# wenhao728/VORTA

Hardware: NVIDIA B200
Metric: dit_denoise_step_ms (lower is better)
Workload: dtype bf16

## Files before the change

include/vorta_b200.h:

```cpp
#ifndef VORTA_B200_H_
#define VORTA_B200_H_

#include <stdint.h>

#ifdef __cplusplus
extern "C" {
#endif

#define VB_OK 0
#define VB_ERR_INVALID (-1)
#define VB_ERR_CUDA (-2)
#define VB_ERR_UNSUPPORTED (-3)

#define VB_BRANCH_FULL 0
#define VB_BRANCH_CORESET 1
#define VB_BRANCH_SLIDING 2
#define VB_BRANCH_SKIP (-1)
#define VB_BRANCH_FULL_LO 3
#define VB_BRANCH_FULL_HI 4
#define VB_BRANCH_FULL_PART(k, n) (16 + 8 * (n) + (k))

#define VB_DTYPE_F32 0
#define VB_DTYPE_BF16 1

// ... 90 lines not shown
int64_t vb_attn_workspace_bytes(const vb_plan* plan, int32_t batch, int32_t heads);
int vb_attn_fwd(vb_plan* plan, const vb_attn_args* args, vb_stream_t stream);

int vb_attn_dense(const void* q, const void* k, const void* v, void* out, const int64_t* q_stride,
                  const int64_t* k_stride, const int64_t* v_stride, const int64_t* out_stride, int32_t batch,
                  int32_t heads, int32_t n_q, int32_t n_k, vb_stream_t stream);

void vb_stats_reset(void);
int64_t vb_stats_launches(void);
double vb_stats_attn_flops(void);

int vb_block_ln_modulate(const void* x, const float* weight, const float* bias, const float* scale, const float* shift,
                         void* out, int64_t rows, int32_t dim, int32_t rows_per_batch, float eps, vb_stream_t stream);
int vb_block_gate_residual(const void* x, const void* y, const float* gate, void* out, int64_t rows, int32_t dim,
                           int32_t rows_per_batch, vb_stream_t stream);
int vb_block_rmsnorm_rope(const void* x, const void* weight, const float* cos_tab, const float* sin_tab, void* out,
                          int64_t rows, int32_t dim, int32_t tokens_per_batch, float eps, vb_stream_t stream);

int vb_block_headnorm_rope(const void* x, const void* weight, const float* cos_tab, const float* sin_tab, void* out,
                           int32_t batch, int32_t rows, int32_t heads, int32_t rope_rows, int32_t dst_rows,
                           int32_t dst_row0, float eps, vb_stream_t stream);

void vb_timing_enable(int on);
int vb_timing_collect(double* kernel_ms, int64_t* launches, double* flops);
#define VB_TIMING_ROUTED 0
#define VB_TIMING_DENSE 1
#define VB_TIMING_KINDS 2
int vb_timing_collect_kinds(double* kernel_ms, int64_t* launches, double* flops);

int vb_ulysses_pack_heads(const void* x, void* send, int32_t s_loc, int32_t heads, int32_t world, int32_t n_tensors,
// ... 18 lines not shown
```

vorta_b200/_lib.py:

```python
from __future__ import annotations

import ctypes as C
import os
import subprocess
from typing import Optional

_HERE = os.path.dirname(os.path.abspath(__file__))
LIB_PATH = os.environ.get("VB_LIB_PATH") or os.path.join(_HERE, "lib", "libvorta_b200.so")
CSRC_DIR = os.path.join(_HERE, "csrc")

VB_OK = 0
VB_ERR_INVALID = -1
VB_ERR_CUDA = -2
VB_ERR_UNSUPPORTED = -3

BRANCH_FULL, BRANCH_CORESET, BRANCH_SLIDING, BRANCH_SKIP = 0, 1, 2, -1
BRANCH_FULL_LO, BRANCH_FULL_HI = 3, 4
DTYPE_F32, DTYPE_BF16 = 0, 1
ATTN_CORESET_KV_FROM_K = 1


def branch_full_part(k: int, n: int) -> int:
    return 16 + 8 * n + k


(PLAN_SEQ_LEN, PLAN_NUM_GROUPS, PLAN_GROUP_SIZE, PLAN_CORESET_LEN, PLAN_NUM_TILES, PLAN_TILE_TOKENS,
 PLAN_NUM_POOLED, PLAN_KEYS_PER_QUERY, PLAN_SLIDING_PAIRS, PLAN_SLIDING_RUNS) = range(10)
(EXPORT_CENTER_INDICES, EXPORT_MARGIN_INDICES, EXPORT_TILE_MAP, EXPORT_TILE_WINDOW, EXPORT_SLIDING_RUNS,
 EXPORT_SLIDING_ITEMS, EXPORT_SLIDING_QUERY_MAP) = range(7)

EXPORTED_SYMBOLS = (
    "vb_last_error", "vb_version", "vb_device_check",
    "vb_plan_create", "vb_plan_destroy", "vb_plan_set_text_valid", "vb_plan_query", "vb_plan_export",
    "vb_router_forward", "vb_coreset_select", "vb_coreset_tables", "vb_gather_rows",
    "vb_attn_workspace_bytes", "vb_attn_fwd", "vb_attn_dense",
    "vb_block_ln_modulate", "vb_block_gate_residual", "vb_block_rmsnorm_rope", "vb_block_headnorm_rope",
    "vb_stats_reset", "vb_stats_launches", "vb_stats_attn_flops", "vb_timing_enable", "vb_timing_collect",
    "vb_timing_collect_kinds",
    "vb_ulysses_pack_heads", "vb_ulysses_pack_qkv", "vb_ulysses_unpack_heads", "vb_ulysses_scatter_qkv_slots",
)


class PlanDesc(C.Structure):
    _fields_ = [
        ("latent", C.c_int32 * 3),
        ("tile", C.c_int32 * 3),
        ("window", C.c_int32 * 3),
        ("lowres_window", C.c_int32 * 3),
        ("n_unpooled", C.c_int32),
        ("text_len", C.c_int32),
        ("text_valid", C.c_int32),
# ... 63 lines not shown
    lib.vb_attn_dense.argtypes = [vp, vp, vp, vp, C.POINTER(i64), C.POINTER(i64), C.POINTER(i64), C.POINTER(i64),
                                  i32, i32, i32, i32, vp]
    lib.vb_gather_rows.restype = C.c_int
    lib.vb_gather_rows.argtypes = [vp, i64, i64, i64, vp, i64, i64, i64, vp, i64, i64, i32, i32, i32, vp]
    lib.vb_attn_workspace_bytes.restype = i64
    lib.vb_attn_workspace_bytes.argtypes = [vp, i32, i32]
    lib.vb_attn_fwd.restype = C.c_int
    lib.vb_attn_fwd.argtypes = [vp, C.POINTER(AttnArgs), vp]
    lib.vb_stats_reset.restype = None
    lib.vb_stats_launches.restype = i64
    lib.vb_stats_attn_flops.restype = C.c_double
    lib.vb_block_ln_modulate.restype = C.c_int
    lib.vb_block_ln_modulate.argtypes = [vp, vp, vp, vp, vp, vp, i64, i32, i32, f32, vp]
    lib.vb_block_gate_residual.restype = C.c_int
    lib.vb_block_gate_residual.argtypes = [vp, vp, vp, vp, i64, i32, i32, vp]
    lib.vb_block_rmsnorm_rope.restype = C.c_int
    lib.vb_block_rmsnorm_rope.argtypes = [vp, vp, vp, vp, vp, i64, i32, i32, f32, vp]
    lib.vb_block_headnorm_rope.restype = C.c_int
    lib.vb_block_headnorm_rope.argtypes = [vp, vp, vp, vp, vp, i32, i32, i32, i32, i32, i32, f32, vp]
    lib.vb_timing_enable.restype = None
    lib.vb_timing_enable.argtypes = [C.c_int]
    lib.vb_timing_collect.restype = C.c_int
    lib.vb_timing_collect.argtypes = [C.POINTER(C.c_double), C.POINTER(i64), C.POINTER(C.c_double)]
    lib.vb_timing_collect_kinds.restype = C.c_int
    lib.vb_timing_collect_kinds.argtypes = [C.POINTER(C.c_double), C.POINTER(i64), C.POINTER(C.c_double)]
    lib.vb_ulysses_pack_heads.restype = C.c_int
    lib.vb_ulysses_pack_heads.argtypes = [vp, vp, i32, i32, i32, i32, i64, i64, C.POINTER(i32), vp]
    lib.vb_ulysses_pack_qkv.restype = C.c_int
    lib.vb_ulysses_pack_qkv.argtypes = [vp, vp, vp, C.POINTER(i64), C.POINTER(i64), vp, i32, i32, i32, C.POINTER(i32), vp]
    lib.vb_ulysses_scatter_qkv_slots.restype = C.c_int
# ... 27 lines not shown
```

vorta_b200/csrc/vb_api.cu:

```cuda
#include <math.h>
#include <stdlib.h>
#include <string.h>

#include <algorithm>
#include <array>
#include <map>
#include <vector>

#include <nvtx3/nvToolsExt.h>

#include "vb_common.cuh"

namespace vb {

struct NvtxRange {
  explicit NvtxRange(const char* name) { nvtxRangePushA(name); }
  ~NvtxRange() { nvtxRangePop(); }
};

static thread_local char g_err[512] = "";
void set_error(const char* fmt, ...) {
  va_list ap;
  va_start(ap, fmt);
  vsnprintf(g_err, sizeof(g_err), fmt, ap);
// ... 13 lines not shown

int launch_coreset_select(const SelectParams& p, cudaStream_t stream);
int launch_gather_rows(const GatherParams& p, cudaStream_t stream);
int launch_coreset_tables(const TablesParams& p, cudaStream_t stream);
int launch_zero_rows(__nv_bfloat16* out, int64_t sb, int64_t sh, int64_t ss, int batch, int heads, int row0,
                     int n_rows, cudaStream_t stream);
int launch_router(const void* temb, int temb_dtype, const void* w, const void* bias, int w_dtype,
                  int64_t w_layer_stride, int64_t bias_layer_stride, int n_layers, int batch, int embed_dim,
                  int heads, float tau, float* scores, int32_t* branch, cudaStream_t stream);
int launch_ulysses_permute(const void* src, void* dst, int s_loc, int heads, int world, int n_tensors,
                           int64_t src_tensor_stride, int64_t dst_tensor_stride, int pack, const int32_t* head_at,
                           cudaStream_t stream);
int launch_ulysses_pack_qkv(const void* q, const void* k, const void* v, const int64_t* stride_s,
                            const int64_t* stride_h, void* send, int s_loc, int heads, int world,
                            const int32_t* head_at, cudaStream_t stream);
int launch_ln_modulate(const void* x, const float* w, const float* b, const float* scale, const float* shift, void* out,
                       int64_t rows, int dim, int rows_per_batch, float eps, cudaStream_t stream);
int launch_gate_residual(const void* x, const void* y, const float* gate, void* out, int64_t rows, int dim,
                         int rows_per_batch, cudaStream_t stream);
int launch_rmsnorm_rope(const void* x, const void* weight, const float* cs, const float* sn, void* out, int64_t rows,
                        int dim, int tokens_per_batch, float eps, cudaStream_t stream);
int launch_headnorm_rope(const void* x, const void* weight, const float* cs, const float* sn, void* out, int batch,
                         int rows, int heads, int rope_rows, int dst_rows, int dst_row0, float eps,
                         cudaStream_t stream);
int launch_ulysses_scatter_slots(const void* q, const void* k, const void* v, const int64_t* stride_s,
                                 const int64_t* stride_h, void* const* peer_qkv, int64_t rows_total, int s_loc, int slots,
                                 int world, int rank, const int32_t* entry_peer, const int32_t* entry_slot,
                                 const int32_t* entry_head, int n_entries, cudaStream_t stream);
int make_qkv_tensor_map(CUtensorMap* map, const void* base, int64_t n_rows, int64_t heads, int64_t batch,
                        int64_t stride_b, int64_t stride_h, int64_t stride_s);
int launch_attn(const AttnTmaps& tmaps, const AttnParams& params, int n_ctas, cudaStream_t stream);

// ... 169 lines not shown
  pl->full.finalize();
  pl->coreset.finalize();
  pl->sliding.finalize();
  if (pl->has_device) {
    int rc;
    if ((rc = pl->full.upload()) != VB_OK) return rc;
    if ((rc = pl->coreset.upload()) != VB_OK) return rc;
    if ((rc = pl->sliding.upload()) != VB_OK) return rc;
  }
  return VB_OK;
}

extern "C" {

const char* vb_last_error(void) { return get_error(); }
int vb_version(void) { return 101; }

int vb_device_check(void) {
  int dev = 0, major = 0, minor = 0, count = 0;
  if (cudaGetDeviceCount(&count) != cudaSuccess || count == 0) {
    cudaGetLastError();
    set_error("no CUDA device: vorta_b200 has no CPU path");
    return VB_ERR_UNSUPPORTED;
  }
  VB_CUDA_OK(cudaGetDevice(&dev));
  VB_CUDA_OK(cudaDeviceGetAttribute(&major, cudaDevAttrComputeCapabilityMajor, dev));
  VB_CUDA_OK(cudaDeviceGetAttribute(&minor, cudaDevAttrComputeCapabilityMinor, dev));
  VB_REQUIRE(major == 10, VB_ERR_UNSUPPORTED, "device is sm_%d%d; this library is built for sm_100a only", major,
             minor);
  return VB_OK;
}
// ... 712 lines not shown
  }
  Output o;
  memset(&o, 0, sizeof(o));
  o.ptr = static_cast<__nv_bfloat16*>(out);
  for (int i = 0; i < 3; ++i) o.stride[i] = out_stride[i];
  Segment sg = segment_of(q, k, v, q_stride, k_stride, v_stride, n_q, n_k, heads, *sched);
  for (int h = 0; h < heads; ++h) sg.heads.push_back(AttnHead{h, h, 0});
  NvtxRange nvtx("vb_attn_dense");
  return launch_segments(&sg, 1, batch, o, nullptr, nullptr, VB_TIMING_DENSE, static_cast<cudaStream_t>(stream_));
}

int vb_block_ln_modulate(const void* x, const float* weight, const float* bias, const float* scale, const float* shift,
                         void* out, int64_t rows, int32_t dim, int32_t rows_per_batch, float eps, vb_stream_t stream) {
  VB_REQUIRE(x && out, VB_ERR_INVALID, "null argument");
  VB_REQUIRE((scale == nullptr) == (shift == nullptr), VB_ERR_INVALID, "scale and shift come together");
  int rc = launch_ln_modulate(x, weight, bias, scale, shift, out, rows, dim, rows_per_batch, eps,
                              static_cast<cudaStream_t>(stream));
  if (rc == VB_OK) ++g_launches;
  return rc;
}
int vb_block_gate_residual(const void* x, const void* y, const float* gate, void* out, int64_t rows, int32_t dim,
                           int32_t rows_per_batch, vb_stream_t stream) {
  VB_REQUIRE(x && y && out, VB_ERR_INVALID, "null argument");
  int rc = launch_gate_residual(x, y, gate, out, rows, dim, rows_per_batch, static_cast<cudaStream_t>(stream));
  if (rc == VB_OK) ++g_launches;
  return rc;
}
int vb_block_rmsnorm_rope(const void* x, const void* weight, const float* cos_tab, const float* sin_tab, void* out,
                          int64_t rows, int32_t dim, int32_t tokens_per_batch, float eps, vb_stream_t stream) {
  VB_REQUIRE(x && weight && out, VB_ERR_INVALID, "null argument");
  VB_REQUIRE((cos_tab == nullptr) == (sin_tab == nullptr), VB_ERR_INVALID, "cos and sin tables come together");
// ... 103 lines not shown
```

vorta_b200/csrc/vb_block.cu:

```cuda
#include "vb_common.cuh"

namespace vb {

constexpr int kRowThreads = 256;
constexpr int kMaxVec = 4;

__device__ __forceinline__ void unpack8(const uint4& v, float (&f)[8]) {
  const uint32_t w[4] = {v.x, v.y, v.z, v.w};
#pragma unroll
  for (int i = 0; i < 4; ++i) {
    f[2 * i + 0] = __uint_as_float(w[i] << 16);
    f[2 * i + 1] = __uint_as_float(w[i] & 0xffff0000u);
  }
}
__device__ __forceinline__ uint32_t pack2(float lo, float hi) {
  uint32_t r;
  asm("cvt.rn.bf16x2.f32 %0, %1, %2;" : "=r"(r) : "f"(hi), "f"(lo));
  return r;
}
__device__ __forceinline__ uint4 pack8(const float (&f)[8]) {
  return make_uint4(pack2(f[0], f[1]), pack2(f[2], f[3]), pack2(f[4], f[5]), pack2(f[6], f[7]));
}
__device__ __forceinline__ void block_sum2(float& a, float& b) {
  __shared__ float red[2][kRowThreads / 32];
#pragma unroll
  for (int o = 16; o >= 1; o >>= 1) {
    a += __shfl_xor_sync(0xffffffffu, a, o);
    b += __shfl_xor_sync(0xffffffffu, b, o);
  }
  const int w = threadIdx.x >> 5, l = threadIdx.x & 31;
  if (l == 0) { red[0][w] = a; red[1][w] = b; }
  __syncthreads();
  a = l < kRowThreads / 32 ? red[0][l] : 0.f;
  b = l < kRowThreads / 32 ? red[1][l] : 0.f;
#pragma unroll
  for (int o = 4; o >= 1; o >>= 1) {
    a += __shfl_xor_sync(0xffffffffu, a, o);
    b += __shfl_xor_sync(0xffffffffu, b, o);
  }
  a = __shfl_sync(0xffffffffu, a, 0);
  b = __shfl_sync(0xffffffffu, b, 0);
  __syncthreads();
}

__global__ void __launch_bounds__(kRowThreads)
vb_ln_modulate_kernel(const __nv_bfloat16* __restrict__ x, const float* __restrict__ w, const float* __restrict__ b,
                      const float* __restrict__ scale, const float* __restrict__ shift, __nv_bfloat16* __restrict__ out,
                      int dim, int rows_per_batch, float eps) {
  const int64_t row = blockIdx.x;
  const int nvec = dim >> 3;
  const uint4* xr = reinterpret_cast<const uint4*>(x + row * dim);
  float v[kMaxVec][8];
  float s1 = 0.f, s2 = 0.f;
#pragma unroll
  for (int i = 0; i < kMaxVec; ++i) {
    const int idx = threadIdx.x + i * kRowThreads;
    if (idx < nvec) {
      unpack8(xr[idx], v[i]);
#pragma unroll
      for (int e = 0; e < 8; ++e) { s1 += v[i][e]; s2 += v[i][e] * v[i][e]; }
    }
  }
  block_sum2(s1, s2);
  const float mean = s1 / dim;
  const float rstd = rsqrtf(fmaxf(s2 / dim - mean * mean, 0.f) + eps);
  const int64_t batch = row / rows_per_batch;
  const float* sc = scale ? scale + batch * dim : nullptr;
  const float* sh = shift ? shift + batch * dim : nullptr;
  uint4* orow = reinterpret_cast<uint4*>(out + row * dim);
#pragma unroll
  for (int i = 0; i < kMaxVec; ++i) {
    const int idx = threadIdx.x + i * kRowThreads;
    if (idx < nvec) {
      float y[8];
#pragma unroll
      for (int e = 0; e < 8; ++e) {
        const int c = idx * 8 + e;
        float t = (v[i][e] - mean) * rstd;
        if (w) t = t * w[c] + (b ? b[c] : 0.f);
        if (sc) t = t * (1.f + sc[c]) + sh[c];
        y[e] = t;
// ... 14 lines not shown
__device__ __forceinline__ float4 ldg4(const float* p) { return __ldg(reinterpret_cast<const float4*>(p)); }

template <int WPR>
__device__ __forceinline__ float row_sum(float a, float (*xchg)[kRowCtaThreads / 32], int slot) {
  a = warp_sum(a);
  if (WPR == 1) return a;
  const int warp = threadIdx.x >> 5, lane = threadIdx.x & 31;
  if (lane == 0) xchg[slot][warp] = a;
  asm volatile("bar.sync %0, %1;" ::"r"(1 + warp / WPR), "r"(32 * WPR) : "memory");
  float r = 0.f;
#pragma unroll
  for (int i = 0; i < WPR; ++i) r += xchg[slot][(warp / WPR) * WPR + i];
  return r;
}

template <int NV>
__global__ void __launch_bounds__(kRowCtaThreads)
vb_ln_modulate_warp_kernel(const __nv_bfloat16* __restrict__ x, const float* __restrict__ w,
                           const float* __restrict__ b, const float* __restrict__ scale,
                           const float* __restrict__ shift, __nv_bfloat16* __restrict__ out, int64_t rows,
                           int rows_per_batch, float eps) {
  constexpr int dim = NV * 256;
  constexpr int WPR = row_warps(NV);
  constexpr int NVT = NV / WPR;
  constexpr int kRowsPerCta = kRowCtaThreads / (32 * WPR);
  __shared__ float xchg[2][kRowCtaThreads / 32];
  const int tid = threadIdx.x & (32 * WPR - 1);
  const int64_t row_raw = static_cast<int64_t>(blockIdx.x) * kRowsPerCta + threadIdx.x / (32 * WPR);
  const bool live = row_raw < rows;
  const int64_t row = live ? row_raw : rows - 1;
  const uint4* xr = reinterpret_cast<const uint4*>(x + row * dim);
  uint4 raw[NVT];
#pragma unroll
  for (int i = 0; i < NVT; ++i) raw[i] = xr[i * 32 * WPR + tid];
  float s1 = 0.f;
#pragma unroll
  for (int i = 0; i < NVT; ++i) {
    float f[8];
    unpack8(raw[i], f);
#pragma unroll
    for (int e = 0; e < 8; ++e) s1 += f[e];
  }
  const float mean = row_sum<WPR>(s1, xchg, 0) * (1.f / dim);
  float s2 = 0.f;
#pragma unroll
  for (int i = 0; i < NVT; ++i) {
    float f[8];
    unpack8(raw[i], f);
#pragma unroll
    for (int e = 0; e < 8; ++e) { const float d = f[e] - mean; s2 = fmaf(d, d, s2); }
  }
  const float rstd = rsqrtf(row_sum<WPR>(s2, xchg, 1) * (1.f / dim) + eps);
  if (!live) return;
  const int64_t batch = row / rows_per_batch;
  const float* sc = scale ? scale + batch * dim : nullptr;
  const float* sh = shift ? shift + batch * dim : nullptr;
  uint4* orow = reinterpret_cast<uint4*>(out + row * dim);
#pragma unroll
  for (int i = 0; i < NVT; ++i) {
    const int c0 = (i * 32 * WPR + tid) * 8;
    float f[8];
    unpack8(raw[i], f);
#pragma unroll
    for (int e = 0; e < 8; ++e) f[e] = (f[e] - mean) * rstd;
    if (w) {
      const float4 w0 = ldg4(w + c0), w1 = ldg4(w + c0 + 4);
      const float wv[8] = {w0.x, w0.y, w0.z, w0.w, w1.x, w1.y, w1.z, w1.w};
      float bv[8] = {0.f, 0.f, 0.f, 0.f, 0.f, 0.f, 0.f, 0.f};
      if (b) {
// ... 65 lines not shown
        const float re = y[2 * pz], im = y[2 * pz + 1];
        y[2 * pz] = re * cv[pz] - im * sv[pz];
        y[2 * pz + 1] = re * sv[pz] + im * cv[pz];
      }
    }
    orow[i * 32 * WPR + tid] = pack8(y);
  }
}

__global__ void __launch_bounds__(256)
vb_gate_residual_kernel(const uint4* __restrict__ x, const uint4* __restrict__ y, const float* __restrict__ gate,
                        uint4* __restrict__ out, int64_t n_vec, int dim, int64_t vec_per_batch) {
  const int dvec = dim >> 3;
  for (int64_t i = static_cast<int64_t>(blockIdx.x) * blockDim.x + threadIdx.x; i < n_vec;
       i += static_cast<int64_t>(gridDim.x) * blockDim.x) {
    float a[8], c[8];
    unpack8(x[i], a);
    unpack8(y[i], c);
    if (gate) {
      const float* g = gate + (i / vec_per_batch) * dim + (i % dvec) * 8;
#pragma unroll
      for (int e = 0; e < 8; ++e) a[e] = fmaf(c[e], g[e], a[e]);
    } else {
#pragma unroll
      for (int e = 0; e < 8; ++e) a[e] += c[e];
    }
    out[i] = pack8(a);
  }
}

__global__ void __launch_bounds__(kRowThreads)
vb_rmsnorm_rope_kernel(const __nv_bfloat16* __restrict__ x, const __nv_bfloat16* __restrict__ weight,
                       const float* __restrict__ cs, const float* __restrict__ sn, __nv_bfloat16* __restrict__ out,
                       int dim, int tokens_per_batch, float eps) {
  const int64_t row = blockIdx.x;
  const int nvec = dim >> 3;
  const uint4* xr = reinterpret_cast<const uint4*>(x + row * dim);
  const uint4* wr = reinterpret_cast<const uint4*>(weight);
  float v[kMaxVec][8];
  float s2 = 0.f, dummy = 0.f;
#pragma unroll
  for (int i = 0; i < kMaxVec; ++i) {
// ... 113 lines not shown
  p.rows = rows; p.heads = heads; p.rope_rows = cs ? rope_rows : 0; p.dst_rows = dst_rows; p.dst_row0 = dst_row0;
  p.eps = eps;
  if (p.units == 0) return VB_OK;
  const int64_t blocks_needed = (p.units / 4 * 16 + 255) / 256 + 1;
  const int grid = static_cast<int>(blocks_needed < 148 * 8 ? blocks_needed : 148 * 8);
  vb_headnorm_rope_kernel<<<grid, 256, 0, stream>>>(p);
  VB_CUDA_OK(cudaGetLastError());
  return VB_OK;
}

static unsigned row_grid(int64_t rows, int nv) {
  const int rows_per_cta = kRowCtaThreads / (32 * row_warps(nv));
  return static_cast<unsigned>((rows + rows_per_cta - 1) / rows_per_cta);
}

int launch_ln_modulate(const void* x, const float* w, const float* b, const float* scale, const float* shift, void* out,
                       int64_t rows, int dim, int rows_per_batch, float eps, cudaStream_t stream) {
  VB_REQUIRE(dim % 8 == 0 && dim <= kRowThreads * kMaxVec * 8, VB_ERR_UNSUPPORTED, "row width %d not supported", dim);
  if (rows == 0) return VB_OK;
  const __nv_bfloat16* xb = static_cast<const __nv_bfloat16*>(x);
  __nv_bfloat16* ob = static_cast<__nv_bfloat16*>(out);
  
  const bool aligned = ((reinterpret_cast<uintptr_t>(w) | reinterpret_cast<uintptr_t>(b) | reinterpret_cast<uintptr_t>(scale) |
                         reinterpret_cast<uintptr_t>(shift)) & 15) == 0;
#define VB_LN_CASE(NV)                                                                                              \
  case NV * 256:                                                                                                    \
    vb_ln_modulate_warp_kernel<NV><<<row_grid(rows, NV), kRowCtaThreads, 0, stream>>>(xb, w, b, scale, shift, ob,  \
                                                                                       rows, rows_per_batch, eps); \
    break;
  switch (aligned ? dim : 0) {
    VB_LN_CASE(4) VB_LN_CASE(6) VB_LN_CASE(8) VB_LN_CASE(12) VB_LN_CASE(16) VB_LN_CASE(20) VB_LN_CASE(24)
    default:
      vb_ln_modulate_kernel<<<static_cast<unsigned>(rows), kRowThreads, 0, stream>>>(xb, w, b, scale, shift, ob, dim,
                                                                                      rows_per_batch, eps);
  }
#undef VB_LN_CASE
  VB_CUDA_OK(cudaGetLastError());
  return VB_OK;
}
int launch_gate_residual(const void* x, const void* y, const float* gate, void* out, int64_t rows, int dim,
                         int rows_per_batch, cudaStream_t stream) {
  VB_REQUIRE(dim % 8 == 0, VB_ERR_UNSUPPORTED, "row width %d not supported", dim);
  const int64_t n_vec = rows * (dim >> 3);
  if (n_vec == 0) return VB_OK;
  const int64_t blocks = (n_vec + 255) / 256;
  const int grid = static_cast<int>(blocks < 148 * 32 ? blocks : 148 * 32);
  vb_gate_residual_kernel<<<grid, 256, 0, stream>>>(static_cast<const uint4*>(x), static_cast<const uint4*>(y), gate,
                                                    static_cast<uint4*>(out), n_vec, dim,
                                                    static_cast<int64_t>(rows_per_batch) * (dim >> 3));
  VB_CUDA_OK(cudaGetLastError());
  return VB_OK;
// ... 30 lines not shown
```

vorta_b200/ops.py:

```python
from __future__ import annotations

import ctypes as C
from typing import Optional, Sequence, Tuple

import numpy as np
import torch

from . import _lib as L

HEAD_DIM = 128


def _stream_ptr(device: torch.device) -> int:
    return torch.cuda.current_stream(device).cuda_stream


def _require_cuda_bf16(name: str, t: torch.Tensor) -> None:
    if not t.is_cuda:
        raise L.VortaB200Error(f"{name} must be a CUDA tensor: vorta_b200 has no CPU path")
    if t.dtype != torch.bfloat16:
        raise ValueError(f"{name} must be bfloat16, got {t.dtype}")
    if t.dim() != 4 or t.shape[-1] != HEAD_DIM or t.stride(-1) != 1:
        raise ValueError(f"{name} must be (B, H, N, {HEAD_DIM}) with contiguous channels, got {tuple(t.shape)} "
                         f"strides {t.stride()}")
# ... 312 lines not shown
def gate_residual(x: torch.Tensor, y: torch.Tensor, gate: Optional[torch.Tensor] = None) -> torch.Tensor:
    x = _contig(x)
    rows, dim, per_batch = _rows(x)
    if y.shape != x.shape:
        raise ValueError("gate_residual: shape mismatch")
    if not y.is_contiguous():
        y = y.contiguous()
    gate = _f32(gate)
    out = torch.empty_like(x)
    with torch.cuda.device(x.device):
        L.check(L.lib().vb_block_gate_residual(x.data_ptr(), y.data_ptr(), gate.data_ptr() if gate is not None else None,
                                               out.data_ptr(), rows, dim, per_batch, _stream_ptr(x.device)))
    return out


def rmsnorm_rope(x: torch.Tensor, weight: torch.Tensor, eps: float, cos: Optional[torch.Tensor] = None,
                 sin: Optional[torch.Tensor] = None) -> torch.Tensor:
    x = _contig(x)
    rows, dim, per_batch = _rows(x)
    w = weight if weight.dtype == torch.bfloat16 and weight.is_contiguous() else weight.to(torch.bfloat16).contiguous()
    out = torch.empty_like(x)
    if cos is not None and (tuple(cos.shape) != (per_batch, HEAD_DIM // 2) or cos.dtype != torch.float32):
        raise ValueError(f"cos / sin tables must be fp32 ({per_batch}, {HEAD_DIM // 2}), got {tuple(cos.shape)}")
    with torch.cuda.device(x.device):
        L.check(L.lib().vb_block_rmsnorm_rope(x.data_ptr(), w.data_ptr(), cos.data_ptr() if cos is not None else None,
                                              sin.data_ptr() if sin is not None else None, out.data_ptr(), rows, dim,
                                              per_batch, float(eps), _stream_ptr(x.device)))
    return out


# ... 33 lines not shown
```

vorta_b200/patch/modeling_hunyuan.py:

```python
from __future__ import annotations

import os
from typing import Any, Dict, Optional, Tuple

import torch
import torch.nn.functional as F

from .. import ops
from ..attention import (HunyuanVideoFlashAttnProcessor, HunyuanVideoFlashAttnProcessorTripleEval,
                         HunyuanVideoFlashAttnProcessorTripleTrain)
from ..ulysses import SP_STATE, all_gather
from .modeling_wan import accumulate_loss, load_router_checkpoint
from .outputs import RoutedTransformerModelOutput
from .router import Router, route_step


def _rotary_1d(dim: int, pos: torch.Tensor, theta: float) -> Tuple[torch.Tensor, torch.Tensor]:
    freqs = 1.0 / (theta ** (torch.arange(0, dim, 2, dtype=torch.float32, device=pos.device)[: dim // 2] / dim))
    ang = torch.outer(pos.float(), freqs)
    return ang.cos().repeat_interleave(2, dim=1), ang.sin().repeat_interleave(2, dim=1)


def hunyuan_rope_forward(self, hidden_states: torch.Tensor) -> Tuple[torch.Tensor, torch.Tensor]:
    _, _, num_frames, height, width = hidden_states.shape
# ... 36 lines not shown
                                      clean_timesteps_emb=None, routing_score=None, branch=None):
    shift_msa, scale_msa, gate_msa, shift_mlp, scale_mlp, gate_mlp = _ada_chunks(self.norm1, temb, 6)
    c_shift_msa, c_scale_msa, c_gate_msa, c_shift_mlp, c_scale_mlp, c_gate_mlp = _ada_chunks(self.norm1_context, temb, 6)
    norm_hidden = ops.ln_modulate(hidden_states, None, None, scale_msa, shift_msa, 1e-6)
    norm_encoder = ops.ln_modulate(encoder_hidden_states, None, None, c_scale_msa, c_shift_msa, 1e-6)
    if use_original_attn:
        attn_out, ctx_out = self.attn(hidden_states=norm_hidden, encoder_hidden_states=norm_encoder,
                                      attention_mask=attention_mask, image_rotary_emb=freqs_cis, use_original_attn=True,
                                      **_text_valid_kw(self_attention_kwargs))
    else:
        if routing_score is None:
            routing_score = self.router(clean_timesteps_emb)
        attn_out, ctx_out = self.attn(hidden_states=norm_hidden, encoder_hidden_states=norm_encoder,
                                      attention_mask=attention_mask, image_rotary_emb=freqs_cis,
                                      **_attn_kwargs(self_attention_kwargs, routing_score, branch))
    hidden_states = ops.gate_residual(hidden_states, attn_out, gate_msa)
    encoder_hidden_states = ops.gate_residual(encoder_hidden_states, ctx_out, c_gate_msa)
    ff = self.ff(ops.ln_modulate(hidden_states, None, None, scale_mlp, shift_mlp, 1e-6))
    ff_ctx = self.ff_context(ops.ln_modulate(encoder_hidden_states, None, None, c_scale_mlp, c_shift_mlp, 1e-6))
    hidden_states = ops.gate_residual(hidden_states, ff, gate_mlp)
    encoder_hidden_states = ops.gate_residual(encoder_hidden_states, ff_ctx, c_gate_mlp)
    return hidden_states, encoder_hidden_states, routing_score


def hunyuan_single_block_routed_forward(self, hidden_states, encoder_hidden_states, temb, attention_mask,
                                        image_rotary_emb, token_replace_emb=None, first_frame_num_tokens: int = 0,
                                        use_original_attn: bool = False, self_attention_kwargs=None,
                                        clean_timesteps_emb=None, routing_score=None, branch=None):
    text_len = encoder_hidden_states.shape[1]
    residual = torch.cat([hidden_states, encoder_hidden_states], dim=1)
    shift, scale, gate = _ada_chunks(self.norm, temb, 3)
    norm = ops.ln_modulate(residual, None, None, scale, shift, 1e-6)
    mlp = torch._addmm_activation(self.proj_mlp.bias, norm.flatten(0, 1), self.proj_mlp.weight.t(),
                                  use_gelu=True).unflatten(0, norm.shape[:2])
    norm_hidden, norm_encoder = norm[:, :-text_len], norm[:, -text_len:]
    if use_original_attn:
        attn_out, ctx_out = self.attn(hidden_states=norm_hidden, encoder_hidden_states=norm_encoder,
                                      attention_mask=attention_mask, image_rotary_emb=image_rotary_emb,
                                      use_original_attn=True, **_text_valid_kw(self_attention_kwargs))
    else:
        if routing_score is None:
            routing_score = self.router(clean_timesteps_emb)
        attn_out, ctx_out = self.attn(hidden_states=norm_hidden, encoder_hidden_states=norm_encoder,
                                      attention_mask=attention_mask, image_rotary_emb=image_rotary_emb,
                                      **_attn_kwargs(self_attention_kwargs, routing_score, branch))
# ... 118 lines not shown
```

vorta_b200/patch/modeling_wan.py:

```python
from __future__ import annotations

import os
from typing import Any, Dict, Optional

import torch
import torch.nn.functional as F

from .. import ops
from ..attention import WanAttnProcessor2_0, WanAttnProcessorTripleEval, WanAttnProcessorTripleTrain
from ..ulysses import SP_STATE, all_gather
from .outputs import RoutedTransformerModelOutput
from .router import Router, route_step


def wan_rope_forward(self, hidden_states: torch.Tensor) -> torch.Tensor:
    _, _, num_frames, height, width = hidden_states.shape
    p_t, p_h, p_w = self.patch_size
    ppf, pph, ppw = num_frames // p_t, height // p_h, width // p_w
    d = self.attention_head_dim
    freqs = self.freqs.to(hidden_states.device).split_with_sizes([d // 2 - 2 * (d // 6), d // 6, d // 6], dim=1)
    f = freqs[0][:ppf].view(ppf, 1, 1, -1).expand(ppf, pph, ppw, -1)
    h = freqs[1][:pph].view(1, pph, 1, -1).expand(ppf, pph, ppw, -1)
    w = freqs[2][:ppw].view(1, 1, ppw, -1).expand(ppf, pph, ppw, -1)
    return torch.cat([f, h, w], dim=-1).reshape(1, 1, ppf * pph * ppw, -1)


def wan_block_routed_forward(self, hidden_states, encoder_hidden_states, temb, rotary_emb,
                             temb_before_proj: Optional[torch.Tensor], use_original_attn: bool = False,
                             self_attention_kwargs: Optional[Dict[str, Any]] = None,
                             routing_score: Optional[torch.Tensor] = None, branch=None):
    shift_msa, scale_msa, gate_msa, c_shift_msa, c_scale_msa, c_gate_msa = (
        t.contiguous() for t in (self.scale_shift_table + temb.float()).unbind(dim=1))

    norm_hidden_states = ops.ln_modulate(hidden_states, None, None, scale_msa, shift_msa, self.norm1.eps)
    if not use_original_attn and routing_score is None:
        routing_score = self.router(temb_before_proj)
    kwargs = dict(self_attention_kwargs or {})
    if branch is not None:
        kwargs["branch"] = branch
    if type(self.attn1.processor) is WanAttnProcessor2_0:
        attn_output = self.attn1(hidden_states=norm_hidden_states, rotary_emb=rotary_emb)
    else:
        attn_output = self.attn1(hidden_states=norm_hidden_states, rotary_emb=rotary_emb, routing_score=routing_score,
                                 use_original_attn=use_original_attn, **kwargs)
    hidden_states = ops.gate_residual(hidden_states, attn_output, gate_msa)

    norm_hidden_states = ops.ln_modulate(hidden_states, self.norm2.weight, self.norm2.bias, None, None, self.norm2.eps)
    attn_output = self.attn2(hidden_states=norm_hidden_states, encoder_hidden_states=encoder_hidden_states)
    hidden_states = ops.gate_residual(hidden_states, attn_output, None)

    norm_hidden_states = ops.ln_modulate(hidden_states, None, None, c_scale_msa, c_shift_msa, self.norm3.eps)
    ff_output = self.ffn(norm_hidden_states)
    hidden_states = ops.gate_residual(hidden_states, ff_output, c_gate_msa)
    return hidden_states, routing_score


def wan_transformer_3d_routed_forward(self, hidden_states: torch.Tensor, timestep: torch.Tensor,
                                      encoder_hidden_states: torch.Tensor,
                                      encoder_hidden_states_image: Optional[torch.Tensor] = None,
                                      return_dict: bool = True, attention_kwargs=None,
                                      self_attention_kwargs: Optional[Dict[str, Any]] = None,
                                      return_losses: bool = False, reture_hidden_layer_distill_loss: bool = False,
                                      return_routing_scores: bool = False):
    batch_size, _, num_frames, height, width = hidden_states.shape
    p_t, p_h, p_w = self.config.patch_size
    ppf, pph, ppw = num_frames // p_t, height // p_h, width // p_w

    rotary_emb = self.rope(hidden_states)
    hidden_states = self.patch_embedding(hidden_states).flatten(2).transpose(1, 2)
# ... 11 lines not shown
    tau = kwargs.get("tau_sparse")
    eval_mode = isinstance(self.blocks[0].attn1.processor, WanAttnProcessorTripleEval)
    dense_baseline = type(self.blocks[0].attn1.processor) is WanAttnProcessor2_0
    if not dense_baseline and not eval_mode and torch.is_grad_enabled() and any(q.requires_grad for q in self.blocks[0].router.parameters()):
        raise NotImplementedError("vorta_b200: router training is not supported yet (no attention backward); run the "
                                  "Train processors under torch.no_grad()")
    reg_loss = hidden_layer_distill_loss = last_layer_distill_loss = None
    if dense_baseline:
        if return_losses or return_routing_scores:
            raise ValueError("the dense baseline (apply_sp_flashattn_transformer) has no routers: no losses / scores")
        scores = branches = None
    else:
        scores, branches = route_step([b.router for b in self.blocks], temb, tau if eval_mode else None)
    self._vb_last_branches = branches if eval_mode else None
    ref_hidden_states = hidden_states.detach().clone() if return_losses else None
    for i, block in enumerate(self.blocks):
        if dense_baseline:
            hidden_states, _ = block(hidden_states, encoder_hidden_states, timestep_proj, rotary_emb,
                                     temb_before_proj=temb, use_original_attn=True)
            continue
        score_i = scores[i].to(temb.dtype)
        hidden_states, _ = block(hidden_states, encoder_hidden_states, timestep_proj, rotary_emb,
                                 temb_before_proj=temb, use_original_attn=False, self_attention_kwargs=kwargs,
                                 routing_score=score_i, branch=branches[i] if eval_mode else None)
        if return_losses:
            with torch.no_grad():
                ref_hidden_states, _ = block(ref_hidden_states, encoder_hidden_states, timestep_proj, rotary_emb,
                                             temb_before_proj=temb, use_original_attn=True)
            reg_loss = accumulate_loss(reg_loss, torch.square(score_i[:, :, 0]).mean().float())
            if reture_hidden_layer_distill_loss:
                hidden_layer_distill_loss = accumulate_loss(
                    hidden_layer_distill_loss, F.mse_loss(ref_hidden_states.float(), hidden_states.float()))
    routing_scores = list(scores.detach().to(temb.dtype).cpu().unbind(0)) if return_routing_scores else []

    shift, scale = ((self.scale_shift_table.float() + temb.float().unsqueeze(1))).unbind(dim=1)
    shift, scale = shift.contiguous(), scale.contiguous()
    hidden_states = self.proj_out(ops.ln_modulate(hidden_states, None, None, scale, shift, self.norm_out.eps))
    if return_losses:
        with torch.no_grad():
            ref_hidden_states = self.proj_out(ops.ln_modulate(ref_hidden_states, None, None, scale, shift,
                                                              self.norm_out.eps))
        last_layer_distill_loss = F.mse_loss(ref_hidden_states.float(), hidden_states.float())
    if SP_STATE.enabled:
        hidden_states = all_gather(hidden_states, dim=1)
    hidden_states = hidden_states.reshape(batch_size, ppf, pph, ppw, p_t, p_h, p_w, -1)
    hidden_states = hidden_states.permute(0, 7, 1, 4, 2, 5, 3, 6)
    output = hidden_states.flatten(6, 7).flatten(4, 5).flatten(2, 3)
    if not return_dict:
        return (output, reg_loss, last_layer_distill_loss, hidden_layer_distill_loss, routing_scores)
    return RoutedTransformerModelOutput(sample=output, reg_loss=reg_loss, last_layer_distill_loss=last_layer_distill_loss,
                                        hidden_layer_distill_loss=hidden_layer_distill_loss,
                                        routing_scores=routing_scores)


def accumulate_loss(current_loss, new_loss):
    return new_loss if current_loss is None else current_loss + new_loss
# ... 44 lines not shown
```

Measured before the change: 3136.

## Fuse gated residual add with following LayerNorm-modulate across DiT blocks

Adds a fused residual+LayerNorm-modulate kernel that computes x + gate*y, writes the updated residual, and produces the normalized, modulated activations in one pass. The Wan block loop is restructured so each block's final gated residual is fused with the next block's norm1 (or the output norm), and the Hunyuan single block avoids a concat when the two sequences are already adjacent in memory. This removes separate elementwise launches and a full extra read of the hidden state per fusion site, at the cost of more complex cross-block plumbing and an extra output buffer.

```diff
diff --git a/include/vorta_b200.h b/include/vorta_b200.h
--- a/include/vorta_b200.h
+++ b/include/vorta_b200.h
@@ -128,6 +128,9 @@
                          void* out, int64_t rows, int32_t dim, int32_t rows_per_batch, float eps, vb_stream_t stream);
 int vb_block_gate_residual(const void* x, const void* y, const float* gate, void* out, int64_t rows, int32_t dim,
                            int32_t rows_per_batch, vb_stream_t stream);
+int vb_block_residual_ln_modulate(const void* x, const void* y, const float* gate, void* x_out, const float* weight,
+                                  const float* bias, const float* scale, const float* shift, void* out, int64_t rows,
+                                  int32_t dim, int32_t rows_per_batch, float eps, vb_stream_t stream);
 int vb_block_rmsnorm_rope(const void* x, const void* weight, const float* cos_tab, const float* sin_tab, void* out,
                           int64_t rows, int32_t dim, int32_t tokens_per_batch, float eps, vb_stream_t stream);
 
diff --git a/vorta_b200/_lib.py b/vorta_b200/_lib.py
--- a/vorta_b200/_lib.py
+++ b/vorta_b200/_lib.py
@@ -34,7 +34,8 @@
     "vb_plan_create", "vb_plan_destroy", "vb_plan_set_text_valid", "vb_plan_query", "vb_plan_export",
     "vb_router_forward", "vb_coreset_select", "vb_coreset_tables", "vb_gather_rows",
     "vb_attn_workspace_bytes", "vb_attn_fwd", "vb_attn_dense",
-    "vb_block_ln_modulate", "vb_block_gate_residual", "vb_block_rmsnorm_rope", "vb_block_headnorm_rope",
+    "vb_block_ln_modulate", "vb_block_gate_residual", "vb_block_residual_ln_modulate", "vb_block_rmsnorm_rope",
+    "vb_block_headnorm_rope",
     "vb_stats_reset", "vb_stats_launches", "vb_stats_attn_flops", "vb_timing_enable", "vb_timing_collect",
     "vb_timing_collect_kinds",
     "vb_ulysses_pack_heads", "vb_ulysses_pack_qkv", "vb_ulysses_unpack_heads", "vb_ulysses_scatter_qkv_slots",
@@ -128,6 +129,8 @@
     lib.vb_block_ln_modulate.argtypes = [vp, vp, vp, vp, vp, vp, i64, i32, i32, f32, vp]
     lib.vb_block_gate_residual.restype = C.c_int
     lib.vb_block_gate_residual.argtypes = [vp, vp, vp, vp, i64, i32, i32, vp]
+    lib.vb_block_residual_ln_modulate.restype = C.c_int
+    lib.vb_block_residual_ln_modulate.argtypes = [vp, vp, vp, vp, vp, vp, vp, vp, vp, i64, i32, i32, f32, vp]
     lib.vb_block_rmsnorm_rope.restype = C.c_int
     lib.vb_block_rmsnorm_rope.argtypes = [vp, vp, vp, vp, vp, i64, i32, i32, f32, vp]
     lib.vb_block_headnorm_rope.restype = C.c_int
diff --git a/vorta_b200/csrc/vb_api.cu b/vorta_b200/csrc/vb_api.cu
--- a/vorta_b200/csrc/vb_api.cu
+++ b/vorta_b200/csrc/vb_api.cu
@@ -51,8 +51,9 @@
 int launch_ulysses_pack_qkv(const void* q, const void* k, const void* v, const int64_t* stride_s,
                             const int64_t* stride_h, void* send, int s_loc, int heads, int world,
                             const int32_t* head_at, cudaStream_t stream);
-int launch_ln_modulate(const void* x, const float* w, const float* b, const float* scale, const float* shift, void* out,
-                       int64_t rows, int dim, int rows_per_batch, float eps, cudaStream_t stream);
+int launch_ln_modulate(const void* x, const void* y, const float* gate, void* x_out, const float* w, const float* b,
+                       const float* scale, const float* shift, void* out, int64_t rows, int dim, int rows_per_batch,
+                       float eps, cudaStream_t stream);
 int launch_gate_residual(const void* x, const void* y, const float* gate, void* out, int64_t rows, int dim,
                          int rows_per_batch, cudaStream_t stream);
 int launch_rmsnorm_rope(const void* x, const void* weight, const float* cs, const float* sn, void* out, int64_t rows,
@@ -252,7 +253,7 @@
 extern "C" {
 
 const char* vb_last_error(void) { return get_error(); }
-int vb_version(void) { return 101; }
+int vb_version(void) { return 102; }
 
 int vb_device_check(void) {
   int dev = 0, major = 0, minor = 0, count = 0;
@@ -995,7 +996,21 @@
                          void* out, int64_t rows, int32_t dim, int32_t rows_per_batch, float eps, vb_stream_t stream) {
   VB_REQUIRE(x && out, VB_ERR_INVALID, "null argument");
   VB_REQUIRE((scale == nullptr) == (shift == nullptr), VB_ERR_INVALID, "scale and shift come together");
-  int rc = launch_ln_modulate(x, weight, bias, scale, shift, out, rows, dim, rows_per_batch, eps,
+  int rc = launch_ln_modulate(x, nullptr, nullptr, nullptr, weight, bias, scale, shift, out, rows, dim, rows_per_batch,
+                              eps, static_cast<cudaStream_t>(stream));
+  if (rc == VB_OK) ++g_launches;
+  return rc;
+}
+int vb_block_residual_ln_modulate(const void* x, const void* y, const float* gate, void* x_out, const float* weight,
+                                  const float* bias, const float* scale, const float* shift, void* out, int64_t rows,
+                                  int32_t dim, int32_t rows_per_batch, float eps, vb_stream_t stream) {
+  VB_REQUIRE(x && y && x_out && out, VB_ERR_INVALID, "null argument");
+  VB_REQUIRE((scale == nullptr) == (shift == nullptr), VB_ERR_INVALID, "scale and shift come together");
+  VB_REQUIRE(out != x && out != y && out != x_out && y != x_out, VB_ERR_INVALID,
+             "residual_ln_modulate: only x_out may alias x");
+  VB_REQUIRE((reinterpret_cast<uintptr_t>(gate) & 15) == 0, VB_ERR_INVALID,
+             "residual_ln_modulate: the gate must be 16-byte aligned");
+  int rc = launch_ln_modulate(x, y, gate, x_out, weight, bias, scale, shift, out, rows, dim, rows_per_batch, eps,
                               static_cast<cudaStream_t>(stream));
   if (rc == VB_OK) ++g_launches;
   return rc;
diff --git a/vorta_b200/csrc/vb_block.cu b/vorta_b200/csrc/vb_block.cu
--- a/vorta_b200/csrc/vb_block.cu
+++ b/vorta_b200/csrc/vb_block.cu
@@ -21,6 +21,25 @@
 __device__ __forceinline__ uint4 pack8(const float (&f)[8]) {
   return make_uint4(pack2(f[0], f[1]), pack2(f[2], f[3]), pack2(f[4], f[5]), pack2(f[6], f[7]));
 }
+__device__ __forceinline__ uint4 residual8(const uint4& xv, const uint4& yv, const float (&g)[8], bool gated) {
+  float a[8], c[8];
+  unpack8(xv, a);
+  unpack8(yv, c);
+  if (gated) {
+#pragma unroll
+    for (int e = 0; e < 8; ++e) a[e] = fmaf(c[e], g[e], a[e]);
+  } else {
+#pragma unroll
+    for (int e = 0; e < 8; ++e) a[e] += c[e];
+  }
+  return pack8(a);
+}
+
+__device__ __forceinline__ void gate8(const float* p, float (&g)[8]) {
+  const float4 a = __ldg(reinterpret_cast<const float4*>(p)), b = __ldg(reinterpret_cast<const float4*>(p) + 1);
+  g[0] = a.x; g[1] = a.y; g[2] = a.z; g[3] = a.w; g[4] = b.x; g[5] = b.y; g[6] = b.z; g[7] = b.w;
+}
+
 __device__ __forceinline__ void block_sum2(float& a, float& b) {
   __shared__ float red[2][kRowThreads / 32];
 #pragma unroll
@@ -43,20 +62,32 @@
   __syncthreads();
 }
 
+template <bool RESIDUAL>
 __global__ void __launch_bounds__(kRowThreads)
-vb_ln_modulate_kernel(const __nv_bfloat16* __restrict__ x, const float* __restrict__ w, const float* __restrict__ b,
+vb_ln_modulate_kernel(const __nv_bfloat16* x, const __nv_bfloat16* __restrict__ y, const float* __restrict__ gate,
+                      __nv_bfloat16* x_out, const float* __restrict__ w, const float* __restrict__ b,
                       const float* __restrict__ scale, const float* __restrict__ shift, __nv_bfloat16* __restrict__ out,
                       int dim, int rows_per_batch, float eps) {
   const int64_t row = blockIdx.x;
   const int nvec = dim >> 3;
   const uint4* xr = reinterpret_cast<const uint4*>(x + row * dim);
+  const int64_t batch = row / rows_per_batch;
   float v[kMaxVec][8];
   float s1 = 0.f, s2 = 0.f;
 #pragma unroll
   for (int i = 0; i < kMaxVec; ++i) {
     const int idx = threadIdx.x + i * kRowThreads;
     if (idx < nvec) {
-      unpack8(xr[idx], v[i]);
+      uint4 xv;
+      if (RESIDUAL) {
+        float gv[8];
+        if (gate) gate8(gate + batch * dim + idx * 8, gv);
+        xv = residual8(xr[idx], __ldg(reinterpret_cast<const uint4*>(y + row * dim) + idx), gv, gate != nullptr);
+        reinterpret_cast<uint4*>(x_out + row * dim)[idx] = xv;
+      } else {
+        xv = __ldg(xr + idx);
+      }
+      unpack8(xv, v[i]);
 #pragma unroll
       for (int e = 0; e < 8; ++e) { s1 += v[i][e]; s2 += v[i][e] * v[i][e]; }
     }
@@ -64,7 +95,6 @@
   block_sum2(s1, s2);
   const float mean = s1 / dim;
   const float rstd = rsqrtf(fmaxf(s2 / dim - mean * mean, 0.f) + eps);
-  const int64_t batch = row / rows_per_batch;
   const float* sc = scale ? scale + batch * dim : nullptr;
   const float* sh = shift ? shift + batch * dim : nullptr;
   uint4* orow = reinterpret_cast<uint4*>(out + row * dim);
@@ -109,9 +139,10 @@
   return r;
 }
 
-template <int NV>
+template <int NV, bool RESIDUAL>
 __global__ void __launch_bounds__(kRowCtaThreads)
-vb_ln_modulate_warp_kernel(const __nv_bfloat16* __restrict__ x, const float* __restrict__ w,
+vb_ln_modulate_warp_kernel(const __nv_bfloat16* x, const __nv_bfloat16* __restrict__ y,
+                           const float* __restrict__ gate, __nv_bfloat16* x_out, const float* __restrict__ w,
                            const float* __restrict__ b, const float* __restrict__ scale,
                            const float* __restrict__ shift, __nv_bfloat16* __restrict__ out, int64_t rows,
                            int rows_per_batch, float eps) {
@@ -125,9 +156,26 @@
   const bool live = row_raw < rows;
   const int64_t row = live ? row_raw : rows - 1;
   const uint4* xr = reinterpret_cast<const uint4*>(x + row * dim);
+  const int64_t batch = row / rows_per_batch;
   uint4 raw[NVT];
-#pragma unroll
-  for (int i = 0; i < NVT; ++i) raw[i] = xr[i * 32 * WPR + tid];
+  if (RESIDUAL) {
+    const uint4* yr = reinterpret_cast<const uint4*>(y + row * dim);
+    uint4 yv[NVT];
+#pragma unroll
+    for (int i = 0; i < NVT; ++i) { raw[i] = xr[i * 32 * WPR + tid]; yv[i] = __ldg(yr + i * 32 * WPR + tid); }
+    uint4* xo = reinterpret_cast<uint4*>(x_out + row * dim);
+#pragma unroll
+    for (int i = 0; i < NVT; ++i) {
+      const int c0 = (i * 32 * WPR + tid) * 8;
+      float gv[8];
+      if (gate) gate8(gate + batch * dim + c0, gv);
+      raw[i] = residual8(raw[i], yv[i], gv, gate != nullptr);
+      if (live) xo[i * 32 * WPR + tid] = raw[i];
+    }
+  } else {
+#pragma unroll
+    for (int i = 0; i < NVT; ++i) raw[i] = __ldg(xr + i * 32 * WPR + tid);
+  }
   float s1 = 0.f;
 #pragma unroll
   for (int i = 0; i < NVT; ++i) {
@@ -147,7 +195,6 @@
   }
   const float rstd = rsqrtf(row_sum<WPR>(s2, xchg, 1) * (1.f / dim) + eps);
   if (!live) return;
-  const int64_t batch = row / rows_per_batch;
   const float* sc = scale ? scale + batch * dim : nullptr;
   const float* sh = shift ? shift + batch * dim : nullptr;
   uint4* orow = reinterpret_cast<uint4*>(out + row * dim);
@@ -243,18 +290,13 @@
   const int dvec = dim >> 3;
   for (int64_t i = static_cast<int64_t>(blockIdx.x) * blockDim.x + threadIdx.x; i < n_vec;
        i += static_cast<int64_t>(gridDim.x) * blockDim.x) {
-    float a[8], c[8];
-    unpack8(x[i], a);
-    unpack8(y[i], c);
+    float g[8];
     if (gate) {
-      const float* g = gate + (i / vec_per_batch) * dim + (i % dvec) * 8;
-#pragma unroll
-      for (int e = 0; e < 8; ++e) a[e] = fmaf(c[e], g[e], a[e]);
-    } else {
-#pragma unroll
-      for (int e = 0; e < 8; ++e) a[e] += c[e];
-    }
-    out[i] = pack8(a);
+      const float* gp = gate + (i / vec_per_batch) * dim + (i % dvec) * 8;
+#pragma unroll
+      for (int e = 0; e < 8; ++e) g[e] = gp[e];
+    }
+    out[i] = residual8(x[i], y[i], g, gate != nullptr);
   }
 }
 
@@ -398,27 +440,41 @@
   return static_cast<unsigned>((rows + rows_per_cta - 1) / rows_per_cta);
 }
 
-int launch_ln_modulate(const void* x, const float* w, const float* b, const float* scale, const float* shift, void* out,
-                       int64_t rows, int dim, int rows_per_batch, float eps, cudaStream_t stream) {
-  VB_REQUIRE(dim % 8 == 0 && dim <= kRowThreads * kMaxVec * 8, VB_ERR_UNSUPPORTED, "row width %d not supported", dim);
-  if (rows == 0) return VB_OK;
-  const __nv_bfloat16* xb = static_cast<const __nv_bfloat16*>(x);
-  __nv_bfloat16* ob = static_cast<__nv_bfloat16*>(out);
-  
+template <bool RESIDUAL>
+static void ln_modulate_dispatch(const __nv_bfloat16* x, const __nv_bfloat16* y, const float* gate,
+                                 __nv_bfloat16* x_out, const float* w, const float* b, const float* scale,
+                                 const float* shift, __nv_bfloat16* out, int64_t rows, int dim, int rows_per_batch,
+                                 float eps, cudaStream_t stream) {
   const bool aligned = ((reinterpret_cast<uintptr_t>(w) | reinterpret_cast<uintptr_t>(b) | reinterpret_cast<uintptr_t>(scale) |
                          reinterpret_cast<uintptr_t>(shift)) & 15) == 0;
 #define VB_LN_CASE(NV)                                                                                              \
   case NV * 256:                                                                                                    \
-    vb_ln_modulate_warp_kernel<NV><<<row_grid(rows, NV), kRowCtaThreads, 0, stream>>>(xb, w, b, scale, shift, ob,  \
-                                                                                       rows, rows_per_batch, eps); \
+    vb_ln_modulate_warp_kernel<NV, RESIDUAL><<<row_grid(rows, NV), kRowCtaThreads, 0, stream>>>(                   \
+        x, y, gate, x_out, w, b, scale, shift, out, rows, rows_per_batch, eps);                                     \
     break;
   switch (aligned ? dim : 0) {
     VB_LN_CASE(4) VB_LN_CASE(6) VB_LN_CASE(8) VB_LN_CASE(12) VB_LN_CASE(16) VB_LN_CASE(20) VB_LN_CASE(24)
     default:
-      vb_ln_modulate_kernel<<<static_cast<unsigned>(rows), kRowThreads, 0, stream>>>(xb, w, b, scale, shift, ob, dim,
-                                                                                      rows_per_batch, eps);
+      vb_ln_modulate_kernel<RESIDUAL><<<static_cast<unsigned>(rows), kRowThreads, 0, stream>>>(
+          x, y, gate, x_out, w, b, scale, shift, out, dim, rows_per_batch, eps);
   }
 #undef VB_LN_CASE
+}
+
+int launch_ln_modulate(const void* x, const void* y, const float* gate, void* x_out, const float* w, const float* b,
+                       const float* scale, const float* shift, void* out, int64_t rows, int dim, int rows_per_batch,
+                       float eps, cudaStream_t stream) {
+  VB_REQUIRE(dim % 8 == 0 && dim <= kRowThreads * kMaxVec * 8, VB_ERR_UNSUPPORTED, "row width %d not supported", dim);
+  if (rows == 0) return VB_OK;
+  const auto* xb = static_cast<const __nv_bfloat16*>(x);
+  const auto* yb = static_cast<const __nv_bfloat16*>(y);
+  auto* xo = static_cast<__nv_bfloat16*>(x_out);
+  auto* ob = static_cast<__nv_bfloat16*>(out);
+  if (y)
+    ln_modulate_dispatch<true>(xb, yb, gate, xo, w, b, scale, shift, ob, rows, dim, rows_per_batch, eps, stream);
+  else
+    ln_modulate_dispatch<false>(xb, nullptr, nullptr, nullptr, w, b, scale, shift, ob, rows, dim, rows_per_batch, eps,
+                                stream);
   VB_CUDA_OK(cudaGetLastError());
   return VB_OK;
 }
diff --git a/vorta_b200/ops.py b/vorta_b200/ops.py
--- a/vorta_b200/ops.py
+++ b/vorta_b200/ops.py
@@ -350,6 +350,30 @@
     return out
 
 
+def residual_ln_modulate(x: torch.Tensor, y: torch.Tensor, gate: Optional[torch.Tensor] = None,
+                         weight: Optional[torch.Tensor] = None, bias: Optional[torch.Tensor] = None,
+                         scale: Optional[torch.Tensor] = None, shift: Optional[torch.Tensor] = None,
+                         eps: float = 1e-6, inplace: bool = False):
+    if inplace and not x.is_contiguous():
+        raise ValueError("residual_ln_modulate: inplace needs a contiguous x")
+    x = _contig(x)
+    rows, dim, per_batch = _rows(x)
+    if y.shape != x.shape:
+        raise ValueError("residual_ln_modulate: shape mismatch")
+    y = _contig(y)
+    gate, weight, bias, scale, shift = _f32(gate), _f32(weight), _f32(bias), _f32(scale), _f32(shift)
+    if gate is not None and gate.data_ptr() % 16:
+        gate = gate.clone()
+    x_out = x if inplace else torch.empty_like(x)
+    h = torch.empty_like(x)
+    p = lambda t: t.data_ptr() if t is not None else None
+    with torch.cuda.device(x.device):
+        L.check(L.lib().vb_block_residual_ln_modulate(x.data_ptr(), y.data_ptr(), p(gate), x_out.data_ptr(), p(weight),
+                                                      p(bias), p(scale), p(shift), h.data_ptr(), rows, dim, per_batch,
+                                                      float(eps), _stream_ptr(x.device)))
+    return x_out, h
+
+
 def rmsnorm_rope(x: torch.Tensor, weight: torch.Tensor, eps: float, cos: Optional[torch.Tensor] = None,
                  sin: Optional[torch.Tensor] = None) -> torch.Tensor:
     x = _contig(x)
diff --git a/vorta_b200/patch/modeling_hunyuan.py b/vorta_b200/patch/modeling_hunyuan.py
--- a/vorta_b200/patch/modeling_hunyuan.py
+++ b/vorta_b200/patch/modeling_hunyuan.py
@@ -74,13 +74,27 @@
         attn_out, ctx_out = self.attn(hidden_states=norm_hidden, encoder_hidden_states=norm_encoder,
                                       attention_mask=attention_mask, image_rotary_emb=freqs_cis,
                                       **_attn_kwargs(self_attention_kwargs, routing_score, branch))
-    hidden_states = ops.gate_residual(hidden_states, attn_out, gate_msa)
-    encoder_hidden_states = ops.gate_residual(encoder_hidden_states, ctx_out, c_gate_msa)
-    ff = self.ff(ops.ln_modulate(hidden_states, None, None, scale_mlp, shift_mlp, 1e-6))
-    ff_ctx = self.ff_context(ops.ln_modulate(encoder_hidden_states, None, None, c_scale_mlp, c_shift_mlp, 1e-6))
+    hidden_states, norm_hidden = ops.residual_ln_modulate(hidden_states, attn_out, gate_msa, None, None, scale_mlp,
+                                                          shift_mlp, 1e-6)
+    encoder_hidden_states, norm_encoder = ops.residual_ln_modulate(encoder_hidden_states, ctx_out, c_gate_msa, None,
+                                                                   None, c_scale_mlp, c_shift_mlp, 1e-6)
+    ff = self.ff(norm_hidden)
+    ff_ctx = self.ff_context(norm_encoder)
     hidden_states = ops.gate_residual(hidden_states, ff, gate_mlp)
     encoder_hidden_states = ops.gate_residual(encoder_hidden_states, ff_ctx, c_gate_mlp)
     return hidden_states, encoder_hidden_states, routing_score
+
+
+def _joint_sequence(hidden_states: torch.Tensor, encoder_hidden_states: torch.Tensor) -> torch.Tensor:
+    B, S, D = hidden_states.shape
+    n = S + encoder_hidden_states.shape[1]
+    if (encoder_hidden_states.shape[0] == B and encoder_hidden_states.shape[2] == D
+            and encoder_hidden_states.dtype == hidden_states.dtype
+            and encoder_hidden_states.untyped_storage().data_ptr() == hidden_states.untyped_storage().data_ptr()
+            and hidden_states.stride() == encoder_hidden_states.stride() == (n * D, D, 1)
+            and encoder_hidden_states.storage_offset() == hidden_states.storage_offset() + S * D):
+        return hidden_states.as_strided((B, n, D), (n * D, D, 1))
+    return torch.cat([hidden_states, encoder_hidden_states], dim=1)
 
 
 def hunyuan_single_block_routed_forward(self, hidden_states, encoder_hidden_states, temb, attention_mask,
@@ -88,7 +102,7 @@
                                         use_original_attn: bool = False, self_attention_kwargs=None,
                                         clean_timesteps_emb=None, routing_score=None, branch=None):
     text_len = encoder_hidden_states.shape[1]
-    residual = torch.cat([hidden_states, encoder_hidden_states], dim=1)
+    residual = _joint_sequence(hidden_states, encoder_hidden_states)
     shift, scale, gate = _ada_chunks(self.norm, temb, 3)
     norm = ops.ln_modulate(residual, None, None, scale, shift, 1e-6)
     mlp = torch._addmm_activation(self.proj_mlp.bias, norm.flatten(0, 1), self.proj_mlp.weight.t(),
diff --git a/vorta_b200/patch/modeling_wan.py b/vorta_b200/patch/modeling_wan.py
--- a/vorta_b200/patch/modeling_wan.py
+++ b/vorta_b200/patch/modeling_wan.py
@@ -29,10 +29,23 @@
                              temb_before_proj: Optional[torch.Tensor], use_original_attn: bool = False,
                              self_attention_kwargs: Optional[Dict[str, Any]] = None,
                              routing_score: Optional[torch.Tensor] = None, branch=None):
-    shift_msa, scale_msa, gate_msa, c_shift_msa, c_scale_msa, c_gate_msa = (
-        t.contiguous() for t in (self.scale_shift_table + temb.float()).unbind(dim=1))
-
-    norm_hidden_states = ops.ln_modulate(hidden_states, None, None, scale_msa, shift_msa, self.norm1.eps)
+    hidden_states, _, routing_score = _wan_block(
+        self, hidden_states, None, encoder_hidden_states, _modulation(self, temb), rotary_emb, temb_before_proj, None,
+        use_original_attn=use_original_attn, self_attention_kwargs=self_attention_kwargs, routing_score=routing_score,
+        branch=branch)
+    return hidden_states, routing_score
+
+
+def _modulation(block, temb: torch.Tensor):
+    return tuple(t.contiguous() for t in (block.scale_shift_table + temb.float()).unbind(dim=1))
+
+
+def _wan_block(self, hidden_states, norm_hidden_states, encoder_hidden_states, modulation, rotary_emb,
+               temb_before_proj, next_norm, use_original_attn: bool = False,
+               self_attention_kwargs: Optional[Dict[str, Any]] = None, routing_score=None, branch=None):
+    shift_msa, scale_msa, gate_msa, c_shift_msa, c_scale_msa, c_gate_msa = modulation
+    if norm_hidden_states is None:
+        norm_hidden_states = ops.ln_modulate(hidden_states, None, None, scale_msa, shift_msa, self.norm1.eps)
     if not use_original_attn and routing_score is None:
         routing_score = self.router(temb_before_proj)
     kwargs = dict(self_attention_kwargs or {})
@@ -43,16 +56,18 @@
     else:
         attn_output = self.attn1(hidden_states=norm_hidden_states, rotary_emb=rotary_emb, routing_score=routing_score,
                                  use_original_attn=use_original_attn, **kwargs)
-    hidden_states = ops.gate_residual(hidden_states, attn_output, gate_msa)
-
-    norm_hidden_states = ops.ln_modulate(hidden_states, self.norm2.weight, self.norm2.bias, None, None, self.norm2.eps)
+    hidden_states, norm_hidden_states = ops.residual_ln_modulate(hidden_states, attn_output, gate_msa, self.norm2.weight,
+                                                                 self.norm2.bias, None, None, self.norm2.eps)
     attn_output = self.attn2(hidden_states=norm_hidden_states, encoder_hidden_states=encoder_hidden_states)
-    hidden_states = ops.gate_residual(hidden_states, attn_output, None)
-
-    norm_hidden_states = ops.ln_modulate(hidden_states, None, None, c_scale_msa, c_shift_msa, self.norm3.eps)
+    hidden_states, norm_hidden_states = ops.residual_ln_modulate(hidden_states, attn_output, None, None, None,
+                                                                 c_scale_msa, c_shift_msa, self.norm3.eps)
     ff_output = self.ffn(norm_hidden_states)
-    hidden_states = ops.gate_residual(hidden_states, ff_output, c_gate_msa)
-    return hidden_states, routing_score
+    if next_norm is None:
+        return ops.gate_residual(hidden_states, ff_output, c_gate_msa), None, routing_score
+    scale, shift, eps = next_norm
+    hidden_states, norm_next = ops.residual_ln_modulate(hidden_states, ff_output, c_gate_msa, None, None, scale, shift,
+                                                        eps)
+    return hidden_states, norm_next, routing_score
 
 
 def wan_transformer_3d_routed_forward(self, hidden_states: torch.Tensor, timestep: torch.Tensor,
@@ -94,32 +109,41 @@
         scores, branches = route_step([b.router for b in self.blocks], temb, tau if eval_mode else None)
     self._vb_last_branches = branches if eval_mode else None
     ref_hidden_states = hidden_states.detach().clone() if return_losses else None
+    shift, scale = ((self.scale_shift_table.float() + temb.float().unsqueeze(1))).unbind(dim=1)
+    out_norm = (scale.contiguous(), shift.contiguous(), self.norm_out.eps)
+    norm_hidden_states = ref_norm_hidden_states = None
+    modulation = _modulation(self.blocks[0], timestep_proj)
     for i, block in enumerate(self.blocks):
+        next_modulation, next_norm = None, out_norm
+        if i + 1 < len(self.blocks):
+            next_modulation = _modulation(self.blocks[i + 1], timestep_proj)
+            next_norm = (next_modulation[1], next_modulation[0], self.blocks[i + 1].norm1.eps)
         if dense_baseline:
-            hidden_states, _ = block(hidden_states, encoder_hidden_states, timestep_proj, rotary_emb,
-                                     temb_before_proj=temb, use_original_attn=True)
-            continue
-        score_i = scores[i].to(temb.dtype)
-        hidden_states, _ = block(hidden_states, encoder_hidden_states, timestep_proj, rotary_emb,
-                                 temb_before_proj=temb, use_original_attn=False, self_attention_kwargs=kwargs,
-                                 routing_score=score_i, branch=branches[i] if eval_mode else None)
+            hidden_states, norm_hidden_states, _ = _wan_block(
+                block, hidden_states, norm_hidden_states, encoder_hidden_states, modulation, rotary_emb, temb,
+                next_norm, use_original_attn=True)
+        else:
+            score_i = scores[i].to(temb.dtype)
+            hidden_states, norm_hidden_states, _ = _wan_block(
+                block, hidden_states, norm_hidden_states, encoder_hidden_states, modulation, rotary_emb, temb,
+                next_norm, use_original_attn=False, self_attention_kwargs=kwargs, routing_score=score_i,
+                branch=branches[i] if eval_mode else None)
         if return_losses:
             with torch.no_grad():
-                ref_hidden_states, _ = block(ref_hidden_states, encoder_hidden_states, timestep_proj, rotary_emb,
-                                             temb_before_proj=temb, use_original_attn=True)
+                ref_hidden_states, ref_norm_hidden_states, _ = _wan_block(
+                    block, ref_hidden_states, ref_norm_hidden_states, encoder_hidden_states, modulation, rotary_emb,
+                    temb, next_norm, use_original_attn=True)
             reg_loss = accumulate_loss(reg_loss, torch.square(score_i[:, :, 0]).mean().float())
             if reture_hidden_layer_distill_loss:
                 hidden_layer_distill_loss = accumulate_loss(
                     hidden_layer_distill_loss, F.mse_loss(ref_hidden_states.float(), hidden_states.float()))
+        modulation = next_modulation
     routing_scores = list(scores.detach().to(temb.dtype).cpu().unbind(0)) if return_routing_scores else []
 
-    shift, scale = ((self.scale_shift_table.float() + temb.float().unsqueeze(1))).unbind(dim=1)
-    shift, scale = shift.contiguous(), scale.contiguous()
-    hidden_states = self.proj_out(ops.ln_modulate(hidden_states, None, None, scale, shift, self.norm_out.eps))
+    hidden_states = self.proj_out(norm_hidden_states)
     if return_losses:
         with torch.no_grad():
-            ref_hidden_states = self.proj_out(ops.ln_modulate(ref_hidden_states, None, None, scale, shift,
-                                                              self.norm_out.eps))
+            ref_hidden_states = self.proj_out(ref_norm_hidden_states)
         last_layer_distill_loss = F.mse_loss(ref_hidden_states.float(), hidden_states.float())
     if SP_STATE.enabled:
         hidden_states = all_gather(hidden_states, dim=1)
```

Result: no change. 3106 (median of 6 runs) (-0.9%).
